# ziyanx02/multiagent-quadruped-environment

Measured on AMD Instinct MI355X. Metric: env-steps/sec (agents x envs x steps/s), go1gate 4096 envs x 2 agents per GPU, higher is better.
Workload: dtype f32 (policy GEMMs and the actuator network's 32 x 32 layer: 2-plane split-f16, 22-bit); 1 GPU; go1gate, 2 agents, num_envs=4096 per GPU (4096 total), 4 substeps x 5 ms per step; parallelism=single GPU

## Files before the change

### multiagent-quadruped-environment_amd/csrc/kernels_physics.hpp

```cpp
#pragma once
#include "mqe_common.hpp"

struct V3 { float x, y, z; };
__device__ __forceinline__ V3 v3(float x, float y, float z) { V3 r; r.x = x; r.y = y; r.z = z; return r; }
__device__ __forceinline__ V3 operator+(V3 a, V3 b) { return v3(a.x + b.x, a.y + b.y, a.z + b.z); }
__device__ __forceinline__ V3 operator-(V3 a, V3 b) { return v3(a.x - b.x, a.y - b.y, a.z - b.z); }
__device__ __forceinline__ V3 operator*(float s, V3 a) { return v3(s * a.x, s * a.y, s * a.z); }
__device__ __forceinline__ float dot(V3 a, V3 b) { return a.x * b.x + a.y * b.y + a.z * b.z; }
__device__ __forceinline__ V3 cross(V3 a, V3 b) { return v3(a.y * b.z - a.z * b.y, a.z * b.x - a.x * b.z, a.x * b.y - a.y * b.x); }
__device__ __forceinline__ V3 ld3(const float* p) { return v3(p[0], p[1], p[2]); }
__device__ __forceinline__ void st3(float* p, V3 a) { p[0] = a.x; p[1] = a.y; p[2] = a.z; }
__device__ __forceinline__ V3 mat_vec(const float* R, V3 v) {
  return v3(R[0] * v.x + R[1] * v.y + R[2] * v.z, R[3] * v.x + R[4] * v.y + R[5] * v.z, R[6] * v.x + R[7] * v.y + R[8] * v.z);
}
__device__ __forceinline__ V3 sym_vec(const float* S, V3 v) {
  return v3(S[0] * v.x + S[3] * v.y + S[4] * v.z, S[3] * v.x + S[1] * v.y + S[5] * v.z, S[4] * v.x + S[5] * v.y + S[2] * v.z);
}

template <int CTRL> __device__ __forceinline__ float dpp_take(float x) {
  return __int_as_float(__builtin_amdgcn_update_dpp(0, __float_as_int(x), CTRL, 0xF, 0xF, true));
}
__device__ __forceinline__ float lane_next(float x) { return dpp_take<0x130>(x); }
__device__ __forceinline__ float lane_prev(float x) { return dpp_take<0x138>(x); }

// ... 208 lines not shown
  float4* c4 = reinterpret_cast<float4*>(cr);
  c4[0] = make_float4(__int_as_float(a), __int_as_float(linkA), __int_as_float(b), __int_as_float(linkB));
  c4[1] = make_float4(p.x, p.y, p.z, sd);
  c4[2] = make_float4(n.x, n.y, n.z, __int_as_float(repA));
  c4[3] = make_float4(0.0f, 0.0f, 0.0f, __int_as_float(repB));
}

__host__ __device__ inline int mqe_maxc_uncapped(int A, int P, int cap_npc) { return 8 * A + cap_npc * P + (A + P > 4 ? 8 : 0); }
__host__ __device__ inline int mqe_maxc(int A, int P, int cap_npc) { const int v = mqe_maxc_uncapped(A, P, cap_npc); return v > 64 ? 64 : v; }
#define MQE_LIMIT_PASSES 4
#define CAP_ROBOT 8

struct PhysLds {
  int root, dof, tau, body, rhs, acc, acth, fcol, leg, legc, basei, sinv, sph, prim, con, side, phi, srec, wacc, total;
};
#define RS_STRIDE 44
#define RS_SLOT 12
#define RS_BIAS 42
#define RS_USN 43
#define RSB_STRIDE 32
#define RSB_INFO 30
__host__ __device__ inline int mqe_maxpair(int maxc) { return maxc / 2; }
__host__ __device__ inline PhysLds phys_lds_layout(int A, int P, int ND, int nbody, int ndof, int nsph, int nprim, int maxc, int rowgs, int pad) {
  const int BODY_STRIDE = BODY_STRIDE_OF(pad), CON_STRIDE = CON_STRIDE_OF(pad);
  PhysLds L; int o = 0;
  L.root = o; o += (A + P) * 13;
  L.dof = o; o += ND * 2;
  L.tau = o; o += 12 * A;
  o = (o + 3) & ~3;
  L.rhs = o; o += (ndof + 3) & ~3;
  L.acc = o; o += (ndof + 3) & ~3;
  L.acth = o; o += 4 * 12 * A;
  L.leg = o; o += A * 4 * LEG_STRIDE;
  L.sinv = o; o += A * 72;
  L.con = o; o += maxc * CON_STRIDE;
  L.body = o; o += nbody * BODY_STRIDE;
  L.phi = L.body; L.srec = L.phi;
  if (rowgs && L.phi + maxc * RS_STRIDE > o) o = L.phi + maxc * RS_STRIDE;
  const int scratch = o;
  L.fcol = o; o += A * 5 * FCOL_STRIDE;
  L.legc = o; o += A * 4 * LEGC_STRIDE;
  L.basei = o; o += A * 24;
  L.sph = scratch; L.prim = scratch + nsph * 4;
  if (L.prim + nprim * 8 > o) o = L.prim + nprim * 8;
  L.side = scratch;
  if (scratch + mqe_maxpair(maxc) * RSB_STRIDE > o) o = scratch + mqe_maxpair(maxc) * RSB_STRIDE;
  L.wacc = scratch + mqe_maxpair(maxc) * RSB_STRIDE;
  if (L.wacc + ((ndof + 3) & ~3) > o) o = L.wacc + ((ndof + 3) & ~3);
  L.total = o;
  return L;
}

__host__ __device__ inline int post_npc_stride(int P) { return (P * 13 + 3) & ~3; }
__host__ __device__ inline int post_staging_floats(int epw, int amp, int nj, int P) { return epw * amp * (MQE_OBS_BAG + 24) + epw * post_npc_stride(P) + epw * nj; }
struct PhysDebug { float* minv; int* nc; float* contacts; int robot; long long* times; int stop_after; };
#define TSTAMP(i) do { if (dbg.times != nullptr && lane == 0) dbg.times[i] = (long long)wall_clock64(); if (dbg.stop_after == (i)) return; } while (0)

enum { PS_LOAD_STATE = 1, PS_LOAD_TAU = 2, PS_STORE_STATE = 4, PS_WRITE_CF = 8 };

enum { PS_F_LINK = 1, PS_F_NPC = 2, PS_F_BOX = 4, PS_F_STATIC = 8,
       PS_F_FEW = 16,
       PS_F_ROW = 32 };
template <int TP> struct ShapeClass {
  static constexpr bool small = TP == 0 || TP == PS_F_LINK || (TP > 0 && (TP & PS_F_FEW) != 0);
  static constexpr int sweep = TP >= 0 ? 1 : -1;
  static constexpr int npq = (small || (TP > 0 && (TP & PS_F_ROW) != 0)) ? 2 : 4;
};
template <int TA, int TP>
struct PhysShape {
  const int A, P, PD, npcdof, ND, nbody, ndof, maxc, n_static;
  const bool has_seesaw, has_box;
  const bool rowgs;
  __device__ __forceinline__ explicit PhysShape(const DevModel* m)
      : A(TA > 0 ? TA : m->A), P(TP == 0 ? 0 : m->P), PD((TP < 0 || (TP & PS_F_NPC)) ? m->n_npc_dyn : 0),
        npcdof((TP < 0 || (TP & PS_F_NPC)) ? m->npc_dofs_each : 0),
        ND((TA > 0 && TP == 0) ? 12 * TA : m->ND), nbody((TA > 0 && TP == 0) ? TA * MQE_NBODY : m->nbody_env),
        ndof((TA > 0 && TP == 0) ? TA * MQE_RD : m->ndof_env), maxc((TA > 0 && TP == 0) ? mqe_maxc(TA, 0, 2) : m->maxc),
        n_static((TP < 0 || (TP & PS_F_STATIC)) ? m->n_static : 0),
        has_seesaw(TP < 0 ? m->has_seesaw != 0 : (TP & PS_F_LINK) != 0), has_box(TP < 0 ? m->has_box != 0 : (TP & PS_F_BOX) != 0),
        rowgs(ShapeClass<TP>::sweep >= 0 ? ShapeClass<TP>::sweep == 1 : m->rowgs != 0) {}
};

template <int TA, int TP, int EPW = 1, bool LATE = false>
__device__ __forceinline__ void phys_substep(const DevModel* __restrict__ m, const DevState& st, float* lds_wave, const int e_first, const int lane_wave,
                                             const int flags, const int no_write, const PhysDebug& dbg, const int hotv,
                                             const DevModel* mtab = nullptr) {
  static_assert(EPW == 1 || (EPW == 2 && TP == 0 && (TA == 1 || TA == 2)), "two envs per wavefront: robot-only scenes of at most two robots");
  auto HI = [&](int i) -> int { return __builtin_amdgcn_readlane(hotv, i); };
  auto HF = [&](int i) -> float { return __int_as_float(__builtin_amdgcn_readlane(hotv, i)); };
  auto HP = [&](int i) -> const float* {
    return as_global(reinterpret_cast<const float*>(((unsigned long long)(unsigned)__builtin_amdgcn_readlane(hotv, i + 1) << 32) | (unsigned long long)(unsigned)__builtin_amdgcn_readlane(hotv, i)));
  };
  auto HMASK = [&]() -> unsigned long long {
    return ((unsigned long long)(unsigned)__builtin_amdgcn_readlane(hotv, HOT_FEAT_MASK_HI) << 32) | (unsigned long long)(unsigned)__builtin_amdgcn_readlane(hotv, HOT_FEAT_MASK_LO);
  };
  constexpr int LW = 64 / EPW;
  const int grp = EPW == 1 ? 0 : lane_wave / LW;
  const int lane = EPW == 1 ? lane_wave : lane_wave - grp * LW;
  const bool evalid = EPW == 1 || e_first + grp < HI(HOT_N);
  const int e = evalid ? e_first + grp : HI(HOT_N) - 1;
  auto gballot = [&](bool p) -> unsigned long long {
    const unsigned long long b = __ballot(p);
    return EPW == 1 ? b : ((b >> (grp * LW)) & ((1ull << (LW & 63)) - 1ull));
  };
  auto wave_max_of_groups = [&](int x) -> int {
    return EPW == 1 ? x : max(__builtin_amdgcn_readlane(x, 0), __builtin_amdgcn_readlane(x, 32));
  };
// ... 1947 lines not shown
        if (ok && h == 0) {
          acthg[nj + jt] = he1; acthg[jt] = err; acthg[3 * nj + jt] = hv1; acthg[2 * nj + jt] = qd;
          ldsg[L.tau + jt] = tau;
          if (ev) {
            ST_LATE(late, st, sub_tau)[((size_t)eg * 4 + (k < 4 ? k : 3)) * nj + jt] = tau;
            if (last) ST_LATE(late, st, torques)[gi] = tau;
            if (lagged) ST_LATE(late, st, lag_buf)[lag_wr] = as;
          }
        }
      }
    }
    __syncthreads();
    if constexpr (TIMED) {
      long long* tt = ST_LATE(late, st, wave_times) + 4 * (size_t)gridDim.x + ((size_t)blockIdx.x * 4 + (k < 4 ? k : 3)) * 16;
      const PhysDebug tdbg = {nullptr, nullptr, nullptr, 0, tt, -1};
      phys_substep<TA, TP, EPW, late>(mk, st, lds_wave, e_first_k, lane_k, last ? (PS_STORE_STATE | PS_WRITE_CF) : 0, 0, tdbg, hotv, ma);
      if (lane_wave == 0) tt[15] = (long long)wall_clock64();
    } else
    phys_substep<TA, TP, EPW, late>(mk, st, lds_wave, e_first_k, lane_k, last ? (PS_STORE_STATE | PS_WRITE_CF) : 0, 0, nodbg, hotv, ma);
    if (evalid)
      for (int jt = glane_k; jt < nj; jt += LW) {
        const float q = lds[L.dof + jt * 2], qd = lds[L.dof + jt * 2 + 1];
        substep_log(ma, ST_LATE(late, st, sub_dof_vel), ST_LATE(late, st, sub_exceed), ((size_t)e_k * 4 + (k < 4 ? k : 3)) * nj + jt, jt % 12, q, qd);
      }
  }
  __syncthreads();
  const int lane_post = late ? lane_wave : lane_run;
  const int lane_pg = EPW == 1 ? lane_post : lane_post - (lane_post / LW) * LW;
  if constexpr (late) {
    st = late_state();
    asm volatile("" : "+s"(e_first_k));
  }
  const int e_post = EPW == 1 ? e_first_k : e;
  if (evalid)
    for (int i = lane_pg; i < 4 * nj; i += LW) {
      const int w = i / nj, jt = i - w * nj;
      st.act_hist[(size_t)w * R12 + (size_t)e_post * nj + jt] = acth[i];
    }
  if constexpr (ShapeClass<TP>::small || TP > 0) if (pa.on) {
    long long* et = nullptr;
    if constexpr (TIMED) { et = st.wave_times + 68 * (size_t)gridDim.x + (size_t)blockIdx.x * 16; if (lane_post == 0) et[0] = (long long)wall_clock64(); }
    __threadfence_block();
    __syncthreads();
    constexpr int AMP = (TA == 1 || TA == 2) ? 2 : MQE_MAX_AGENTS;
    float* sb = lds_wave + L.body;
    float* act_l = sb + EPW * AMP * (MQE_OBS_BAG + 24) + EPW * post_npc_stride(P);
    for (int i = lane_post; i < EPW * nj; i += 64) {
      const int ge = i / nj, jt = i - ge * nj;
      if (e_first + ge < m->N) act_l[ge * nj + jt] = st.actions[(size_t)(e_first + ge) * nj + jt];
    }
    __syncthreads();
    if constexpr (TIMED) { if (lane_post == 0) et[1] = (long long)wall_clock64(); }
    post_body<AMP, EPW, true>(m, st, (int)blockIdx.x, lane_post, sb, sb + EPW * AMP * MQE_OBS_BAG, sb + EPW * AMP * (MQE_OBS_BAG + 24), pa.wrapper_level, pa.push_count, pa.step_no,
                        lds_wave + L.root, lds_wave + L.dof, act_l, L.total, nj, post_npc_stride(P), et);
    if constexpr (TIMED) { if (lane_post == 0) et[10] = (long long)wall_clock64(); }
  }
  if (st.wave_times && lane_post == 0) st.wave_times[4 * blockIdx.x + 1] = (long long)wall_clock64();
}
```

### multiagent-quadruped-environment_amd/csrc/kernels_step.hpp

```cpp
#pragma once
#include <type_traits>
#include "mqe_common.hpp"

__device__ __forceinline__ void quat_rotate_inverse_f(const float* q, const float* v, float* o) {
  float qw = q[3];
  float s = 2.0f * qw * qw - 1.0f;
  float cx = q[1] * v[2] - q[2] * v[1], cy = q[2] * v[0] - q[0] * v[2], cz = q[0] * v[1] - q[1] * v[0];
  float dt = q[0] * v[0] + q[1] * v[1] + q[2] * v[2];
  o[0] = v[0] * s - cx * qw * 2.0f + q[0] * dt * 2.0f;
  o[1] = v[1] * s - cy * qw * 2.0f + q[1] * dt * 2.0f;
  o[2] = v[2] * s - cz * qw * 2.0f + q[2] * dt * 2.0f;
}
__device__ __forceinline__ float wrap2pi(float a) {
  const float T = 6.2831855f;
  float r = fmodf(a, T);
  if (r < 0) r += T;
  return r;
}
__device__ __forceinline__ void euler_xyz_f(const float* q, float* rpy) {
  float x = q[0], y = q[1], z = q[2], w = q[3];
  float sinr = 2.0f * (w * x + y * z), cosr = w * w - x * x - y * y + z * z;
  float sinp = 2.0f * (w * y - z * x);
  float siny = 2.0f * (w * z + x * y), cosy = w * w + x * x - y * y - z * z;
  float roll = atan2f(sinr, cosr);
// ... 482 lines not shown
typedef const __attribute__((address_space(3))) float* lds_cptr;
template <class NP>
__device__ __forceinline__ void sheep_flock_mean(const DevModel* m, NP npc_rows, float* avg) {
  const int P = m->P;
  avg[0] = 0; avg[1] = 0; avg[2] = 0;
  for (int p = 0; p < P; p++) for (int k = 0; k < 3; k++) avg[k] += npc_rows[p * 13 + k];
  for (int k = 0; k < 3; k++) avg[k] /= (float)P;
}
template <class NP>
__device__ __forceinline__ void sheep_flock_stats(const DevModel* m, const DevState& st, int e, NP npc_rows, const float* avg) {
  const int P = m->P;
  float var = 0;
  for (int k = 0; k < 2; k++) {
    float acc = 0;
    for (int p = 0; p < P; p++) { float t = npc_rows[p * 13 + k] - avg[k]; acc += t * t; }
    var += acc / (float)P;
  }
  st.sheep_avg[e * 2] = avg[0]; st.sheep_avg[e * 2 + 1] = avg[1];
  st.sheep_var[e] = var;
}
template <class NP, class RP>
__device__ __forceinline__ void sheep_increment(const DevModel* m, const DevState& st, int e, int p, NP npc_rows, RP rob_rows, const float* avg, int step_no, float* dv) {
  const int A = m->A, P = m->P;
  NP sp = npc_rows + p * 13;
  for (int k = 0; k < 3; k++) {
    const float z = m->noise_mode == MQE_NOISE_SCRIPTED ? st.npc_noise[((size_t)e * P + p) * 3 + k]
                                                        : (m->sheep_rand != 0.0f ? mqe_randn(m, e, step_no, (uint32_t)(p * 3 + k)) : 0.0f);
    dv[k] = m->sheep_rand * z * 2.0f;
  }
  if (P != 1) {
    float rel[3] = {avg[0] - sp[0], avg[1] - sp[1], avg[2] - sp[2]};
    float nr = sqrtf(rel[0] * rel[0] + rel[1] * rel[1] + rel[2] * rel[2]);
    if (nr > 0.0f) for (int k = 0; k < 3; k++) dv[k] += m->sheep_rand * rel[k] / nr / 1.5f;
  }
  for (int a = 0; a < A; a++) {
    RP dp = rob_rows + a * 13;
    float rel[3] = {sp[0] - dp[0], sp[1] - dp[1], sp[2] - dp[2]};
    float sq[3] = {rel[0] * rel[0], rel[1] * rel[1], rel[2] * rel[2]};
    float dis = sqrtf(sq[0] * sq[0] + sq[1] * sq[1] + sq[2] * sq[2]);
    float den = powf(dis, 1.4f);
    for (int k = 0; k < 3; k++) { float t = rel[k] / den; if (dis > 9.0f) t = 0.0f; dv[k] += m->sheep_scale * t; }
  }
  dv[2] = 0.0f;
}
template <class NP>
__device__ __forceinline__ void sheep_apply(float* root, int A, int p, NP npc_rows, const float* dv) {
  float* sp = root + (A + p) * 13;
  NP old = npc_rows + p * 13;
  const float v0 = clampf(old[7] + dv[0], -2.0f, 2.0f), v1 = clampf(old[8] + dv[1], -2.0f, 2.0f), v2 = old[9] + dv[2];
  sp[7] = v0; sp[8] = v1; sp[9] = v2;
  sp[2] = clampf(old[2], 0.0f, 0.3f);
  sp[3] = 0.0f; sp[4] = 0.0f;
}
template <bool BAG_LDS = false>
__device__ __forceinline__ void wrapper_env_dev(const DevModel* m, const DevState& st, int e, int is_reset_call, const float* npc, int side_effects = 1, const float* bag_in = nullptr) {
  typedef typename std::conditional<BAG_LDS, const __attribute__((address_space(3))) float*, const float*>::type bag_ptr;
  bag_ptr bag;
  if constexpr (BAG_LDS) bag = (bag_ptr)bag_in;
  else bag = bag_in ? bag_in : st.obs_bag + (size_t)e * m->A * MQE_OBS_BAG;
  int A = m->A, P = m->P, Aw = m->Aw, D = m->D;
  const int task = m->task;
  float* obs = st.wobs + (size_t)e * Aw * D;
  float* rew = st.wrew + (size_t)e * Aw;
  float* rs = st.rsum + (size_t)e * MQE_MAX_REWARD_TERMS;
  float sc[7];
#pragma unroll
  for (int k = 0; k < 7; k++) sc[k] = m->reward_scale[k];
  const bool early = task == MQE_TASK_GATE || task == MQE_TASK_SHEEP || task == MQE_TASK_SEESAW || task == MQE_TASK_PUSHBOX || task == MQE_TASK_FOOTBALL_DEFENDER;
  float gp0 = 0.0f, gp1 = 0.0f, eol[3] = {0.0f, 0.0f, 0.0f}, eo0 = 0.0f, eo1 = 0.0f;
  if (task == MQE_TASK_GATE || task == MQE_TASK_SHEEP || task == MQE_TASK_PUSHBOX || (task == MQE_TASK_FOOTBALL_DEFENDER && !is_reset_call && (sc[0] != 0 || sc[1] != 0))) {
    gp0 = as_global(m->gate_pos)[e * 2]; gp1 = as_global(m->gate_pos)[e * 2 + 1];
  }
  if (task == MQE_TASK_PUSHBOX || task == MQE_TASK_FOOTBALL_DEFENDER)
    for (int k = 0; k < 3; k++) eol[k] = st.env_origins_live[e * 3 + k];
  if (task == MQE_TASK_SHEEP) { eo0 = as_global(m->env_origins)[e * 3]; eo1 = as_global(m->env_origins)[e * 3 + 1]; }
  if (early) {
    if (is_reset_call) { for (int a = 0; a < Aw; a++) rew[a] = 0; }
    else {
      float r_env = 0.0f;
      uint8_t was_reset = st.reset_buf[e];
      float rsv[7];
#pragma unroll
      for (int k = 0; k < 7; k++) rsv[k] = rs[k];
      if (task == MQE_TASK_GATE) {
        float r_ag[MQE_MAX_AGENTS] = {0, 0, 0, 0}, bx[MQE_MAX_AGENTS] = {0, 0, 0, 0}, by[MQE_MAX_AGENTS] = {0, 0, 0, 0}, wl[MQE_MAX_AGENTS] = {0, 0, 0, 0};
        const uint8_t have = st.w_have_last[e];
        const float gx = gp0, colf = (float)st.collide_buf[e];
        float rs0 = rsv[0], rs1 = rsv[1], rs2 = rsv[2], rs3 = rsv[3];
        const float wp0 = m->wrapper_param[0], wp1 = m->wrapper_param[1];
#pragma unroll
        for (int a = 0; a < MQE_MAX_AGENTS; a++)
          if (a < A) {
            bag_ptr ob = bag + (a) * MQE_OBS_BAG;
            bx[a] = ob[0]; by[a] = ob[1];
            wl[a] = st.w_last[e * MQE_MAX_AGENTS + a];
          }
        float tsum = 0;
#pragma unroll
        for (int a = 0; a < MQE_MAX_AGENTS; a++)
          if (a < A) {
            const float tx = wp0, ty = (a == 0 ? 1.0f : -1.0f) * wp1;
            const float dist = sqrtf((bx[a] - tx) * (bx[a] - tx) + (by[a] - ty) * (by[a] - ty));
            const float last = have ? wl[a] : dist;
            tsum += last - dist;
            st.w_last[e * MQE_MAX_AGENTS + a] = dist;
          }
        st.w_have_last[e] = 1;
// ... 66 lines not shown
        for (int a = 0; a < MQE_MAX_AGENTS; a++) if (a < A) wl[a] = st.w_last[e * MQE_MAX_AGENTS + a];
#pragma unroll
        for (int a = 0; a < MQE_MAX_AGENTS; a++)
          if (a < A) {
            bag_ptr ob = bag + (a) * MQE_OBS_BAG;
            const float x = ob[0];
            xs += x - (have ? wl[a] : x);
            st.w_last[e * MQE_MAX_AGENTS + a] = x;
            zs += ob[2]; y2 += ob[1] * ob[1];
          }
        st.w_have_last[e] = 1;
        if (sc[0] != 0) { if (was_reset) xs = 0; xs *= sc[0]; r_env += xs; rsv[0] += xs; }
        if (sc[1] != 0) { float v = sc[1] * (zs - 0.56f); r_env += v; rsv[1] += v; }
        if (sc[2] != 0) { float v = sc[2] * (y2 - 0.5f); r_env += v; rsv[2] += v; }
        if (sc[3] != 0) { float v = sc[3] * colf; r_env += v; rsv[3] += v; }
        if (sc[4] != 0) {
          bag_ptr o0 = bag; bag_ptr o1 = bag + (A - 1) * MQE_OBS_BAG;
          float d2 = (o0[0] - o1[0]) * (o0[0] - o1[0]) + (o0[1] - o1[1]) * (o0[1] - o1[1]);
          if (d2 < 0.25f) { float v = div_ieee(sc[4], d2); r_env += v; rsv[4] += v; }
        }
        if (sc[5] != 0) {
          int cnt = 0;
          for (int a = 0; a < A; a++) { bag_ptr ob = bag + (a) * MQE_OBS_BAG; if (ob[0] > 7.7f && ob[2] > 1.3f) cnt++; }
          float v = sc[5] * (float)cnt; r_env += v; rsv[5] += v;
        }
        if (fell) { r_env += sc[6]; rsv[6] += sc[6]; }
        for (int a = 0; a < Aw; a++) rew[a] = r_env;
      } else if (task == MQE_TASK_PUSHBOX) {
        const float bx = npc[0] - eol[0], wl20 = st.w_last2[e * 2];
        const uint8_t have = st.w_have_last[e];
        if (sc[0] != 0 && have) {
          float xm = bx - wl20;
          if (was_reset) xm = 0;
          const float v = sc[0] * xm;
          r_env += v; rsv[0] += v;
        }
        st.w_last2[e * 2] = bx;
        st.w_have_last[e] = 1;
        for (int a = 0; a < Aw; a++) rew[a] = r_env;
      } else if (task == MQE_TASK_FOOTBALL_DEFENDER) {
        float bx = npc[0] - eol[0], by = npc[1] - eol[1];
        if (sc[0] != 0) { if (bx > gp0) { r_env += sc[0]; rsv[0] += sc[0]; } }
        if (sc[1] != 0) {
          float dg = sqrtf((bx - gp0) * (bx - gp0) + (by - gp1) * (by - gp1));
          float v = sc[1] * expf(-dg / 3.0f);
          r_env += v; rsv[1] += v;
        }
        for (int a = 0; a < Aw; a++) rew[a] = r_env;
      }
#pragma unroll
      for (int k = 0; k < 7; k++) rs[k] = rsv[k];
    }
  }
  for (int a = 0; a < Aw; a++) {
    float* o = obs + a * D;
    int c = 0;
    if (task == MQE_TASK_TUG) {
      const float npos = st.dof[((size_t)e * m->ND + 12 * A) * 2], nvel = st.dof[((size_t)e * m->ND + 12 * A) * 2 + 1];
      const float sgn = a == 1 ? -1.0f : 1.0f;
      bag_ptr ob = bag + (a) * MQE_OBS_BAG;
      float v6[6];
      for (int k = 0; k < 6; k++) v6[k] = ob[k];
      const float dx = v6[0] - 1.6f, dy = v6[1] - npos;
      v6[1] *= sgn; v6[4] *= sgn;
      for (int k = 0; k < 6; k++) o[k] = v6[k];
      o[6] = sgn * npos; o[7] = nvel; o[8] = sqrtf(dx * dx + dy * dy); o[9] = sgn * npos;
      continue;
    }
    if (task != MQE_TASK_ROTATION && task != MQE_TASK_BRIDGE && task != MQE_TASK_WRESTLING)
      for (int k = 0; k < Aw; k++) o[c++] = (k == a) ? 1.0f : 0.0f;
    bag_ptr ob = bag + (a) * MQE_OBS_BAG;
    for (int k = 0; k < 6; k++) o[c++] = ob[k];
    if (task != MQE_TASK_PLAIN) {
      bag_ptr ob2 = bag + ((Aw - 1 - a)) * MQE_OBS_BAG;
      for (int k = 0; k < 6; k++) o[c++] = ob2[k];
    }
    if (task == MQE_TASK_GATE || task == MQE_TASK_SHEEP || task == MQE_TASK_PUSHBOX) { o[c++] = gp0; o[c++] = gp1; }
    if (task == MQE_TASK_PUSHBOX) {
      o[c++] = npc[0] - eol[0]; o[c++] = npc[1] - eol[1];
      for (int k = 0; k < 4; k++) o[c++] = npc[3 + k];
    }
    if (task == MQE_TASK_SHEEP)
      for (int p = 0; p < P; p++) { o[c++] = npc[p * 13] - eo0; o[c++] = npc[p * 13 + 1] - eo1; }
    if (task == MQE_TASK_FOOTBALL_DEFENDER) {
      for (int k = 0; k < 3; k++) o[c++] = npc[k] - eol[k];
      for (int k = 0; k < 3; k++) o[c++] = npc[7 + k];
    }
  }
  if (early) return;
  if (task == MQE_TASK_TUG) {
    float* nd = st.dof + ((size_t)e * m->ND + 12 * A) * 2;
    const float npos = nd[0];
    bag_ptr ob0 = bag;
    bag_ptr ob1 = bag + (1) * MQE_OBS_BAG;
    const float x0 = ob0[0], y0 = ob0[1], x1 = ob1[0], y1 = ob1[1];
    if (is_reset_call) {
      st.w_last[e * MQE_MAX_AGENTS] = x0; st.w_last[e * MQE_MAX_AGENTS + 1] = y0;
      st.w_last2[e * 2] = npos;
      st.w_delayed_reset[e] = 0;
      for (int a = 0; a < Aw; a++) rew[a] = 0;
      return;
    }
    const float last_npc = st.w_last2[e * 2];
    const float lx = st.w_last[e * MQE_MAX_AGENTS] - 1.6f, ly = st.w_last[e * MQE_MAX_AGENTS + 1] - npos;
    const float cx = x0 - 1.6f, cy = y0 - npos;
    const float last_dis = sqrtf(lx * lx + ly * ly), dis = sqrtf(cx * cx + cy * cy);
    float r0 = 0.0f, sr = 0.0f, pu = 0.0f, pr = 0.0f, pp = 0.0f;
    if (sc[0] != 0) { if (npos < 0) sr = sc[0] * -npos; if (last_npc <= npos) sr /= 2; r0 += sr; rs[0] += sr; }
    if (sc[1] != 0) { if (npos > 0) pu = sc[1] * npos; if (last_npc > npos) pu /= 2; r0 -= pu; rs[1] += pu; }
    if (sc[2] != 0) { if (dis < last_dis) pr = (last_dis - dis) * sc[2]; r0 += pr; rs[2] += pr; }
    if (sc[3] != 0) { if (dis >= last_dis) pp = powf(2.0f, dis) * sc[3]; r0 -= pp; rs[3] += pp; }
    rs[4] += npos; rs[5] += pr + sr - pu; rs[6] += x0; rs[7] += y0; rs[8] += x1; rs[9] += y1;
    st.w_last[e * MQE_MAX_AGENTS] = x0; st.w_last[e * MQE_MAX_AGENTS + 1] = y0;
    st.w_last2[e * 2] = npos;
    rew[0] = r0;
    for (int a = 1; a < Aw; a++) rew[a] = 0;
    if (side_effects) {
      uint8_t cnt = st.reset_buf[e] ? 2 : st.w_delayed_reset[e];
      if (cnt > 0) { nd[0] = 0.0f; nd[1] = 0.0f; cnt--; }
      st.w_delayed_reset[e] = cnt;
    }
    return;
  }
  if (task == MQE_TASK_BRIDGE) {
    bag_ptr ob0 = bag;
    bag_ptr ob1 = bag + (1) * MQE_OBS_BAG;
    const float x0 = ob0[0], z0 = ob0[2], x1 = ob1[0], z1 = ob1[2];
    float S = st.w_last[e * MQE_MAX_AGENTS], tgt = st.w_last[e * MQE_MAX_AGENTS + 1];
    if (is_reset_call) {
      S = fabsf(x1 + x0); tgt = x1;
      st.w_last[e * MQE_MAX_AGENTS] = S; st.w_last[e * MQE_MAX_AGENTS + 1] = tgt;
    }
    float* o1 = obs + 1 * D;
    o1[0] = S - o1[0]; o1[4] = -o1[4]; o1[6] = S - o1[6]; o1[10] = -o1[10];
    if (is_reset_call) { for (int a = 0; a < Aw; a++) rew[a] = 0; return; }
    float r0 = 0.0f;
    if (sc[0] != 0 && z1 < 0.5f) { r0 += sc[0]; rs[0] += sc[0]; }
    if (sc[1] != 0 && z0 < 0.5f) { r0 -= sc[1]; rs[1] += sc[1]; }
    if (sc[2] != 0 && x0 > tgt) { r0 += sc[2]; rs[2] += sc[2]; }
    rew[0] = r0;
    for (int a = 1; a < Aw; a++) rew[a] = 0;
    return;
  }
  if (task == MQE_TASK_WRESTLING) {
    float* o1 = obs + 1 * D;
    o1[1] = -o1[1]; o1[4] = -o1[4]; o1[7] = -o1[7]; o1[10] = -o1[10];
    if (is_reset_call) { for (int a = 0; a < Aw; a++) rew[a] = 0; return; }
    float r0 = 0.0f;
    bool down0, down1;
    {
      bag_ptr ob = bag;
      float r = ob[3], p = ob[4];
      if (r > 3.1415927f) r -= 6.2831855f;
      if (p > 3.1415927f) p -= 6.2831855f;
      down0 = fabsf(p) > 3.1415927f * 0.9f || fabsf(r) >= 3.1415927f * 0.4f;
      ob += MQE_OBS_BAG;
      r = ob[3]; p = ob[4];
      if (r > 3.1415927f) r -= 6.2831855f;
      if (p > 3.1415927f) p -= 6.2831855f;
      down1 = fabsf(p) > 3.1415927f * 0.9f || fabsf(r) >= 3.1415927f * 0.4f;
    }
    if (sc[0] != 0 && down1) { r0 += sc[0]; rs[0] += sc[0]; }
    if (sc[1] != 0 && down0) { r0 -= sc[1]; rs[1] += sc[1]; }
    rew[0] = r0;
    for (int a = 1; a < Aw; a++) rew[a] = 0;
    return;
  }
  if (task == MQE_TASK_ROTATION) {
    float* o1 = obs + 1 * D;
    o1[1] = -o1[1]; o1[4] = -o1[4]; o1[7] = -o1[7]; o1[10] = -o1[10];
    const float tgt = m->wrapper_param[0];
    bag_ptr ob0 = bag;
    bag_ptr ob1 = bag + (1) * MQE_OBS_BAG;
    const float x0 = ob0[0], y0 = ob0[1], x1 = ob1[0];
    if (is_reset_call) {
      st.w_last[e * MQE_MAX_AGENTS] = sqrtf((x0 - tgt) * (x0 - tgt) + y0 * y0);
      for (int a = 0; a < Aw; a++) rew[a] = 0;
      return;
    }
    float r0 = 0.0f;
    if (sc[0] != 0 && x0 > tgt) { r0 += sc[0]; rs[0] += sc[0]; }
    if (sc[1] != 0 && x1 > tgt) { r0 -= sc[1]; rs[1] += sc[1]; }
    if (sc[2] != 0) {
      const float dis = sqrtf((x0 - tgt) * (x0 - tgt) + (y0 - tgt) * (y0 - tgt));
      if (dis < st.w_last[e * MQE_MAX_AGENTS]) { r0 += sc[2]; rs[2] += sc[2]; }
      st.w_last[e * MQE_MAX_AGENTS] = dis;
    }
    rew[0] = r0;
    for (int a = 1; a < Aw; a++) rew[a] = 0;
    return;
  }
  for (int a = 0; a < Aw; a++) rew[a] = 0;
}

#ifndef POST_EPW
#define POST_EPW 8
#endif

__device__ __forceinline__ void post_flush_rows(float* __restrict__ g, const float* lds, const int n, const int tid) {
  const int n4 = n >> 2;
  for (int i = tid; i < n4; i += 64) reinterpret_cast<float4*>(g)[i] = reinterpret_cast<const float4*>(lds)[i];
  for (int i = (n4 << 2) + tid; i < n; i += 64) g[i] = lds[i];
}

template <int AM, int PEPW, bool LDS_STATE = false>
__device__ __forceinline__ void post_body(const DevModel* m, const DevState& st, const int blk, const int tid, float* s_bag, float* s_la, float* s_npc,
                                          int wrapper_level, int push_count, int step_no,
                                          const float* root_l = nullptr, const float* dof_l = nullptr, const float* act_l = nullptr, int lds_env_stride = 0, int act_env_stride = 0,
                                          const int npc_stride = MQE_MAX_NPCS * 13, long long* taps = nullptr) {
  static_assert(PEPW * AM <= 64 && (PEPW & (PEPW - 1)) == 0, "agent lanes of PEPW envs must fit one wavefront");
#define ETAP(i) do { if (taps != nullptr && tid == 0) taps[i] = (long long)wall_clock64(); } while (0)
  const int A = m->A, P = m->P;
  const int le = tid & (PEPW - 1), a = tid / PEPW;
  const int e = blk * PEPW + le;
  const bool mine = e < m->N && a < A;
  const bool lead = e < m->N && a == 0;
  const int i = e * A + a;
  const int nrow = min(PEPW, m->N - blk * PEPW) * A;
  const float dtp = m->dt * (float)m->decimation;
  float* root = st.root + (size_t)e * (A + P) * 13;
  float* bag = s_bag + le * A * MQE_OBS_BAG;
  typedef typename std::conditional<LDS_STATE, lds_cptr, const float*>::type state_ptr;
  state_ptr root_src;
  if constexpr (LDS_STATE) root_src = (lds_cptr)(root_l + le * lds_env_stride); else root_src = root;
  float* la = s_la + le * A * 12;
  float rs[13], gpar[5], gi0 = 0.f, f3[3], aoz = 0.f, dq[24], act[12], eo[3];
  int ep = 0;
  if (mine) {
    ep = st.ep_len[e] + 1;
#pragma unroll
    for (int k = 0; k < 3; k++) eo[k] = as_global(m->env_origins)[e * 3 + k];
#pragma unroll
    for (int k = 0; k < 13; k++) rs[k] = root_src[a * 13 + k];
    const float* lo = st.loco_obs + (size_t)i * MQE_FRAME;
#pragma unroll
    for (int k = 0; k < 5; k++) gpar[k] = lo[7 + k];
    gi0 = st.gait[i];
    const float* cf3 = st.cf + ((size_t)e * m->NBR + a * MQE_NREP) * 3;
#pragma unroll
    for (int k = 0; k < 3; k++) f3[k] = cf3[k];
    aoz = as_global(m->agent_origins)[(size_t)i * 3 + 2];
    state_ptr ds, as;
    if constexpr (LDS_STATE) { ds = (lds_cptr)(dof_l + le * lds_env_stride + a * 24); as = (lds_cptr)(act_l + le * act_env_stride + a * 12); }
    else { ds = st.dof + ((size_t)e * m->ND + a * 12) * 2; as = st.actions + (size_t)i * 12; }
#pragma unroll
    for (int k = 0; k < 24; k++) dq[k] = ds[k];
#pragma unroll
    for (int k = 0; k < 12; k++) act[k] = as[k];
  }
  float bq[4], lv[3], av[3], pgr[3], clk[4], gi1 = 0.f;
  float rpy[3] = {0.f, 0.f, 0.f};
  unsigned fl = 0;
  if (mine) {
#pragma unroll
    for (int k = 0; k < 4; k++) bq[k] = rs[3 + k];
    fl = robot_frame(m, rs, gpar, gi0, f3, aoz, dtp, lv, av, pgr, clk, gi1, rpy);
  }
  ETAP(2);
#pragma unroll
  for (int d = PEPW; d < PEPW * AM; d <<= 1) fl |= (unsigned)__shfl_xor((int)fl, d);
  const uint8_t to = ep > m->max_episode_length;
  const uint8_t reset = (uint8_t)(mine && (fl != 0 || to));
  if (lead) env_flags_store(m, st, e, ep, fl, to, reset);
  if (mine) robot_frame_store(st, i, lv, av, pgr, bq, clk, gi1);
  ETAP(3);
  float* npc_pre = s_npc + le * npc_stride;
  {
    const int e0 = blk * PEPW, nenv = min(PEPW, m->N - e0), per = P * 13;
    for (int t = tid; t < nenv * per; t += 64) {
      const int sl = t / per, r = t - sl * per;
      if constexpr (LDS_STATE) s_npc[sl * npc_stride + r] = ((lds_cptr)(root_l + sl * lds_env_stride))[A * 13 + r];
      else s_npc[sl * npc_stride + r] = st.root[((size_t)(e0 + sl) * (A + P) + A) * 13 + r];
    }
    __syncthreads();
  }
  ETAP(4);
  if (m->npc_kind == MQE_NPC_SHEEP) {
    constexpr int LPE = 64 / PEPW, NPASS = (MQE_MAX_NPCS + LPE - 1) / LPE;
    float dvs[NPASS][3];
    if (e < m->N) {
      float avg[3];
      sheep_flock_mean(m, (lds_cptr)npc_pre, avg);
      if (lead) sheep_flock_stats(m, st, e, (lds_cptr)npc_pre, avg);
#pragma unroll
      for (int q = 0; q < NPASS; q++)
        if (a + q * LPE < P) sheep_increment(m, st, e, a + q * LPE, (lds_cptr)npc_pre, root_src, avg, step_no, dvs[q]);
    }
    __syncthreads();
    if (e < m->N) {
#pragma unroll
      for (int q = 0; q < NPASS; q++)
        if (a + q * LPE < P) sheep_apply(root, A, a + q * LPE, (lds_cptr)npc_pre, dvs[q]);
    }
    __threadfence_block();
    __syncthreads();
  }
  ETAP(5);
  if (lead) {
    if (reset) {
      reset_env_dev(m, st, e);
      for (int k = 0; k < P * 13; k++) npc_pre[k] = root[A * 13 + k];
    }
  }
  if (__ballot(reset != 0)) {
    __threadfence_block();
    __syncthreads();
    if (reset) {
#pragma unroll
      for (int k = 0; k < 13; k++) rs[k] = root[a * 13 + k];
      const float* ds = st.dof + ((size_t)e * m->ND + a * 12) * 2;
#pragma unroll
      for (int k = 0; k < 24; k++) dq[k] = ds[k];
      if (P == 0) {
#pragma unroll
        for (int k = 0; k < 4; k++) { bq[k] = rs[3 + k]; st.bquat[i * 4 + k] = bq[k]; }
        euler_xyz_f(bq, rpy);
      }
    }
  }
  ETAP(6);
  if (mine) {
    float* ob = bag + a * MQE_OBS_BAG;
#pragma unroll
    for (int k = 0; k < 3; k++) obs_row_axis(ob, k, rs[k], eo[k], rpy[k], lv[k], av[k], pgr[k]);
#pragma unroll
    for (int j = 0; j < 12; j++) obs_row_joint(m, ob, j, dq[2 * j], dq[2 * j + 1], act[j], act[j]);
#pragma unroll
    for (int k = 0; k < 4; k++) obs_row_quad(ob, k, clk[k], bq[k]);
#pragma unroll
    for (int k = 71; k < MQE_OBS_BAG; k++) ob[k] = 0.0f;
#pragma unroll
    for (int j = 0; j < 12; j++) {
      la[a * 12 + j] = act[j];
      la[PEPW * AM * 12 + a * 12 + j] = dq[2 * j + 1];
    }
  }
  __syncthreads();
  ETAP(7);
  if (lead) {
    wrapper_env_dev<true>(m, st, e, 0, npc_pre, wrapper_level, bag);
    if (push_count > 0 && !reset) push_robots(m, root, e, A, push_count);
  }
  ETAP(8);
  {
    const size_t r0 = (size_t)blk * PEPW * A;
    post_flush_rows(st.obs_bag + r0 * MQE_OBS_BAG, s_bag, nrow * MQE_OBS_BAG, tid);
    post_flush_rows(st.last_actions + r0 * 12, s_la, nrow * 12, tid);
    post_flush_rows(st.last_dof_vel + r0 * 12, s_la + PEPW * AM * 12, nrow * 12, tid);
  }
  ETAP(9);
  unsigned long long rm = __ballot(lead && reset != 0);
  while (rm) {
    const int l = __ffsll((long long)rm) - 1;
    rm &= rm - 1;
    zero_env_history(m, st, blk * PEPW + l, tid, 64);
  }
}

template <int AM>
__global__ void __launch_bounds__(64) k_post_physics(const DevModel* m, DevState st, int wrapper_level, int push_count, int step_no) {
  __shared__ float4 s_bag4[POST_EPW * AM * MQE_OBS_BAG / 4], s_la4[POST_EPW * AM * 24 / 4];
  __shared__ float s_npc[POST_EPW * MQE_MAX_NPCS * 13];
  post_body<AM, POST_EPW>(m, st, blockIdx.x, threadIdx.x, reinterpret_cast<float*>(s_bag4), reinterpret_cast<float*>(s_la4), s_npc, wrapper_level, push_count, step_no);
}

__global__ void k_reset_history(const DevModel* m, DevState st) {
  int idx = blockIdx.x * blockDim.x + threadIdx.x;
  int i = idx / HIST_F4;
  if (i >= m->R) return;
  if (!st.reset_buf[i / m->A]) return;
  reinterpret_cast<float4*>(st.hist)[idx] = make_float4(0.f, 0.f, 0.f, 0.f);
  if (st.hist2) {
    const int w = idx - i * HIST_F4;
    if (w < HIST2_U4) reinterpret_cast<uint4*>(st.hist2)[(size_t)i * HIST2_U4 + w] = make_uint4(0u, 0u, 0u, 0u);
    if (w == 0) st.hist_irr[i] = 0u;
  }
}

__global__ void k_hist2_rebuild(const DevModel* m, DevState st, int oldest) {
  const int idx = blockIdx.x * blockDim.x + threadIdx.x;
  const int i = idx / MQE_HIST, slot = idx - i * MQE_HIST;
  if (i >= m->R || !st.hist2) return;
  const float* fr = st.hist + ((size_t)i * MQE_HIST + slot) * MQE_FRAME;
  uint16_t* row2 = st.hist2 + (size_t)i * (2 * MQE_HIST * MQE_H2_FRAME);
  unsigned any = 0u;
  for (int c = 0; c < 70; c++) {
    const float v = fr[c];
    any |= __float_as_uint(v) & 0x7FFFFFFFu;
    const int cc = h2_col(c);
    if (cc >= 0) {
      uint16_t h, l;
      split2(v, MQE_H2_ASCALE, h, l);
      const size_t k = (size_t)slot * MQE_H2_FRAME + cc;
// ... 96 lines not shown
```

### multiagent-quadruped-environment_amd/csrc/mqe_common.hpp

```cpp
#pragma once
#include <hip/hip_runtime.h>
#include <stdint.h>
#include <string.h>
#include <stddef.h>
#include <type_traits>

#include "../../include/mqe_hip.h"

#define MQE_RD 18
#define MQE_OBS_BAG 74
#define MQE_WAVE 64

struct DevMlp {
  int n_layers;
  int dims[MQE_MAX_LAYERS + 1];
  const float* W[MQE_MAX_LAYERS];
  const float* b[MQE_MAX_LAYERS];
};

struct DevModel {
  int N, A, P, R, ND, NBR, Aw, D;
  int npc_kind, task, npc_dofs_each, npc_lin_only, n_npc_dyn;
  int env_id_offset, seed, noise_mode;
  float dt; int decimation; float gravity_z; int solver_iterations;
  float contact_offset, max_depen, friction, erp;
  int solver_type, vel_iters;
  mqe_robot_model robot;
  float npc_mass, npc_inertia; int npc_n_spheres; float npc_sphere_center[8][3]; float npc_sphere_radius[8];
  int self_collision;
  int rowgs;
  int lag_steps; float max_push;
  int has_box, cap_npc; float npc_box_half[3];
  float seesaw_default_angle;
  int n_static; float sb_center[4][3], sb_half[4][3];
  int has_seesaw, ss_axis, ss_link_cyl; float ss_joint_offset[3], ss_plank_center[3], ss_plank_half[3], ss_base_half[3];
  float ss_inertia, ss_vel_limit, ss_col_radius, ss_col_length, ss_theta_lo, ss_theta_hi;
  int control_type; float action_scale, hip_scale_reduction, clip_actions; float torque_limits[12]; float kp, kd;
  float default_dof_pos[12]; float command_obs[70]; float cmd_lin_scale, cmd_ang_scale; int clip_command;
  int cmd_dims, cmd_general; int cmd_src[18]; float cmd_scale[18];
  const float* wall_sdf; int sdf_nx, sdf_ny; float hs, wall_height, ground_z;
  const float* wall_top;
  const float* wall_corner;
  int edge_mask;
  float prim_feat_t[MQE_MAX_PRIMS][2];
  const float* ground_height;
  float soft_lo[12], soft_hi[12];
  const float *env_origins, *agent_origins, *base_init, *npc_init, *gate_pos;
  int curriculum, terrain_rows, terrain_cols; float terrain_env_length;
  const float* terrain_origins; const int32_t* terrain_types;
  int termination_flags, terminate_on_base_contact, max_episode_length;
  float roll_thr, pitch_thr, zlow_thr, zhigh_thr;
  float dof_ratio_lo, dof_ratio_hi; int has_base_pos_range, has_npc_pos_range;
  float base_pos_x_lo, base_pos_x_hi, base_pos_y_lo, base_pos_y_hi, npc_pos_x_lo, npc_pos_x_hi, npc_pos_y_lo, npc_pos_y_hi;
  float base_vel_lo, base_vel_hi;
  float sheep_scale, sheep_rand;
  float reward_scale[MQE_MAX_REWARD_TERMS]; float wrapper_param[8];
  uint32_t hot[64];
  DevMlp actuator;
  const float* act_frag;
  const uint16_t* act_frag16; int act_f16;
  int nbody_env, ndof_env, nsph_env, nprim_env, maxc;
  unsigned long long feat_sphere_mask;
};

// ... 225 lines not shown
```

Measured before the change: 40.19 million env-steps/s.

## Spread post-step observation rows and wrapper obs across all wavefront lanes

In the LDS-state post path, each agent lane now stashes its per-agent frame quantities into a small LDS record. Afterwards all 64 lanes build the observation-bag rows cooperatively, one axis, joint or quad row call per lane, instead of one agent lane doing every row. The wrapper's per-agent observation assembly is also moved out of the single lead lane into a lane-parallel function, and the lead lane skips that loop. This trades extra LDS staging, an added barrier and index arithmetic for removing the serial per-lane work that left most of the wavefront idle.

```diff
diff --git a/multiagent-quadruped-environment_amd/csrc/kernels_physics.hpp b/multiagent-quadruped-environment_amd/csrc/kernels_physics.hpp
--- a/multiagent-quadruped-environment_amd/csrc/kernels_physics.hpp
+++ b/multiagent-quadruped-environment_amd/csrc/kernels_physics.hpp
@@ -284,7 +284,8 @@
 }
 
 __host__ __device__ inline int post_npc_stride(int P) { return (P * 13 + 3) & ~3; }
-__host__ __device__ inline int post_staging_floats(int epw, int amp, int nj, int P) { return epw * amp * (MQE_OBS_BAG + 24) + epw * post_npc_stride(P) + epw * nj; }
+__host__ __device__ inline int post_rec_offset(int epw, int amp, int nj, int P) { return epw * amp * (MQE_OBS_BAG + 24) + epw * post_npc_stride(P) + epw * nj; }
+__host__ __device__ inline int post_staging_floats(int epw, int amp, int nj, int P) { return post_rec_offset(epw, amp, nj, P) + epw * amp * MQE_POST_REC; }
 struct PhysDebug { float* minv; int* nc; float* contacts; int robot; long long* times; int stop_after; };
 #define TSTAMP(i) do { if (dbg.times != nullptr && lane == 0) dbg.times[i] = (long long)wall_clock64(); if (dbg.stop_after == (i)) return; } while (0)
 
@@ -2338,7 +2339,7 @@
     __syncthreads();
     if constexpr (TIMED) { if (lane_post == 0) et[1] = (long long)wall_clock64(); }
     post_body<AMP, EPW, true>(m, st, (int)blockIdx.x, lane_post, sb, sb + EPW * AMP * MQE_OBS_BAG, sb + EPW * AMP * (MQE_OBS_BAG + 24), pa.wrapper_level, pa.push_count, pa.step_no,
-                        lds_wave + L.root, lds_wave + L.dof, act_l, L.total, nj, post_npc_stride(P), et);
+                        lds_wave + L.root, lds_wave + L.dof, act_l, L.total, nj, post_npc_stride(P), et, sb + post_rec_offset(EPW, AMP, nj, P));
     if constexpr (TIMED) { if (lane_post == 0) et[10] = (long long)wall_clock64(); }
   }
   if (st.wave_times && lane_post == 0) st.wave_times[4 * blockIdx.x + 1] = (long long)wall_clock64();
diff --git a/multiagent-quadruped-environment_amd/csrc/kernels_step.hpp b/multiagent-quadruped-environment_amd/csrc/kernels_step.hpp
--- a/multiagent-quadruped-environment_amd/csrc/kernels_step.hpp
+++ b/multiagent-quadruped-environment_amd/csrc/kernels_step.hpp
@@ -558,7 +558,7 @@
   sp[2] = clampf(old[2], 0.0f, 0.3f);
   sp[3] = 0.0f; sp[4] = 0.0f;
 }
-template <bool BAG_LDS = false>
+template <bool BAG_LDS = false, bool OBS_ON_LANES = false>
 __device__ __forceinline__ void wrapper_env_dev(const DevModel* m, const DevState& st, int e, int is_reset_call, const float* npc, int side_effects = 1, const float* bag_in = nullptr) {
   typedef typename std::conditional<BAG_LDS, const __attribute__((address_space(3))) float*, const float*>::type bag_ptr;
   bag_ptr bag;
@@ -731,7 +731,7 @@
       for (int k = 0; k < 7; k++) rs[k] = rsv[k];
     }
   }
-  for (int a = 0; a < Aw; a++) {
+  for (int a = 0; a < (OBS_ON_LANES ? 0 : Aw); a++) {
     float* o = obs + a * D;
     int c = 0;
     if (task == MQE_TASK_TUG) {
@@ -811,7 +811,7 @@
       st.w_last[e * MQE_MAX_AGENTS] = S; st.w_last[e * MQE_MAX_AGENTS + 1] = tgt;
     }
     float* o1 = obs + 1 * D;
-    o1[0] = S - o1[0]; o1[4] = -o1[4]; o1[6] = S - o1[6]; o1[10] = -o1[10];
+    if constexpr (!OBS_ON_LANES) { o1[0] = S - o1[0]; o1[4] = -o1[4]; o1[6] = S - o1[6]; o1[10] = -o1[10]; }
     if (is_reset_call) { for (int a = 0; a < Aw; a++) rew[a] = 0; return; }
     float r0 = 0.0f;
     if (sc[0] != 0 && z1 < 0.5f) { r0 += sc[0]; rs[0] += sc[0]; }
@@ -823,7 +823,7 @@
   }
   if (task == MQE_TASK_WRESTLING) {
     float* o1 = obs + 1 * D;
-    o1[1] = -o1[1]; o1[4] = -o1[4]; o1[7] = -o1[7]; o1[10] = -o1[10];
+    if constexpr (!OBS_ON_LANES) { o1[1] = -o1[1]; o1[4] = -o1[4]; o1[7] = -o1[7]; o1[10] = -o1[10]; }
     if (is_reset_call) { for (int a = 0; a < Aw; a++) rew[a] = 0; return; }
     float r0 = 0.0f;
     bool down0, down1;
@@ -847,7 +847,7 @@
   }
   if (task == MQE_TASK_ROTATION) {
     float* o1 = obs + 1 * D;
-    o1[1] = -o1[1]; o1[4] = -o1[4]; o1[7] = -o1[7]; o1[10] = -o1[10];
+    if constexpr (!OBS_ON_LANES) { o1[1] = -o1[1]; o1[4] = -o1[4]; o1[7] = -o1[7]; o1[10] = -o1[10]; }
     const float tgt = m->wrapper_param[0];
     bag_ptr ob0 = bag;
     bag_ptr ob1 = bag + (1) * MQE_OBS_BAG;
@@ -872,9 +872,67 @@
   for (int a = 0; a < Aw; a++) rew[a] = 0;
 }
 
+template <int PEPW>
+__device__ __forceinline__ void wrapper_obs_lanes(const DevModel* m, const DevState& st, const int blk, const int tid, const float* s_bag, const float* s_npc, const int npc_stride) {
+  static_assert(PEPW <= 2 && MQE_MAX_AGENTS == 4, "env and agent of an element are found by comparisons");
+  const int A = m->A, P = m->P, Aw = m->Aw, D = m->D, task = m->task;
+  const int e0 = blk * PEPW, nenv = min(PEPW, m->N - e0), per = Aw * D;
+  const bool mirrored = task == MQE_TASK_ROTATION || task == MQE_TASK_BRIDGE || task == MQE_TASK_WRESTLING;
+  const int c_own = mirrored ? 0 : Aw, c_other = c_own + 6, c_task = task == MQE_TASK_PLAIN ? c_other : c_other + 6;
+  for (int idx = tid; idx < nenv * per; idx += 64) {
+    const int sl = (PEPW > 1 && idx >= per) ? 1 : 0;
+    const int i2 = idx - sl * per;
+    const int a = (i2 >= D ? 1 : 0) + (i2 >= 2 * D ? 1 : 0) + (i2 >= 3 * D ? 1 : 0);
+    const int c = i2 - a * D, e = e0 + sl;
+    lds_cptr bag = (lds_cptr)(s_bag + sl * A * MQE_OBS_BAG);
+    lds_cptr npc = (lds_cptr)(s_npc + sl * npc_stride);
+    float v = 0.0f;
+    bool have = true;
+    if (task == MQE_TASK_TUG) {
+      const float* nd = st.dof + ((size_t)e * m->ND + 12 * A) * 2;
+      const float npos = nd[0], sgn = a == 1 ? -1.0f : 1.0f;
+      lds_cptr ob = bag + a * MQE_OBS_BAG;
+      if (c < 6) { v = ob[c]; if (c == 1 || c == 4) v *= sgn; }
+      else if (c == 6 || c == 9) v = sgn * npos;
+      else if (c == 7) v = nd[1];
+      else if (c == 8) { const float dx = ob[0] - 1.6f, dy = ob[1] - npos; v = sqrtf(dx * dx + dy * dy); }
+      else have = false;
+    } else if (c < c_own) v = (c == a) ? 1.0f : 0.0f;
+    else if (c < c_task) {
+      v = c < c_other ? bag[a * MQE_OBS_BAG + (c - c_own)] : bag[(Aw - 1 - a) * MQE_OBS_BAG + (c - c_other)];
+      if (mirrored && a == 1) {
+        if (task == MQE_TASK_BRIDGE) {
+          if (c == 0 || c == 6) v = st.w_last[e * MQE_MAX_AGENTS] - v;
+          else if (c == 4 || c == 10) v = -v;
+        } else if (c == 1 || c == 4 || c == 7 || c == 10) v = -v;
+      }
+    } else {
+      int k = c - c_task;
+      have = false;
+      if (task == MQE_TASK_GATE || task == MQE_TASK_SHEEP || task == MQE_TASK_PUSHBOX) {
+        if (k < 2) { v = as_global(m->gate_pos)[e * 2 + k]; have = true; }
+        k -= 2;
+      }
+      if (!have && task == MQE_TASK_PUSHBOX) {
+        if (k < 2) { v = npc[k] - st.env_origins_live[e * 3 + k]; have = true; }
+        else if (k < 6) { v = npc[3 + (k - 2)]; have = true; }
+      }
+      if (!have && task == MQE_TASK_SHEEP && k < 2 * P) { v = npc[(k >> 1) * 13 + (k & 1)] - as_global(m->env_origins)[e * 3 + (k & 1)]; have = true; }
+      if (!have && task == MQE_TASK_FOOTBALL_DEFENDER) {
+        if (k < 3) { v = npc[k] - st.env_origins_live[e * 3 + k]; have = true; }
+        else if (k < 6) { v = npc[7 + (k - 3)]; have = true; }
+      }
+    }
+    if (have) st.wobs[(size_t)e * per + i2] = v;
+  }
+}
+
 #ifndef POST_EPW
 #define POST_EPW 8
 #endif
+
+struct PostRec { enum { EO = 0, POS = 3, RPY = 6, LV = 9, AV = 12, PG = 15, CLK = 18, BQ = 22, USED = 26 }; };
+static_assert(PostRec::USED <= MQE_POST_REC && MQE_POST_REC % 4 == 0, "the record keeps the staging area's 16 B granules");
 
 __device__ __forceinline__ void post_flush_rows(float* __restrict__ g, const float* lds, const int n, const int tid) {
   const int n4 = n >> 2;
@@ -886,8 +944,10 @@
 __device__ __forceinline__ void post_body(const DevModel* m, const DevState& st, const int blk, const int tid, float* s_bag, float* s_la, float* s_npc,
                                           int wrapper_level, int push_count, int step_no,
                                           const float* root_l = nullptr, const float* dof_l = nullptr, const float* act_l = nullptr, int lds_env_stride = 0, int act_env_stride = 0,
-                                          const int npc_stride = MQE_MAX_NPCS * 13, long long* taps = nullptr) {
+                                          const int npc_stride = MQE_MAX_NPCS * 13, long long* taps = nullptr,
+                                          float* s_rec = nullptr) {
   static_assert(PEPW * AM <= 64 && (PEPW & (PEPW - 1)) == 0, "agent lanes of PEPW envs must fit one wavefront");
+  static_assert(!LDS_STATE || PEPW <= 2, "the element lanes find their env by one comparison");
 #define ETAP(i) do { if (taps != nullptr && tid == 0) taps[i] = (long long)wall_clock64(); } while (0)
   const int A = m->A, P = m->P;
   const int le = tid & (PEPW - 1), a = tid / PEPW;
@@ -919,13 +979,14 @@
 #pragma unroll
     for (int k = 0; k < 3; k++) f3[k] = cf3[k];
     aoz = as_global(m->agent_origins)[(size_t)i * 3 + 2];
-    state_ptr ds, as;
-    if constexpr (LDS_STATE) { ds = (lds_cptr)(dof_l + le * lds_env_stride + a * 24); as = (lds_cptr)(act_l + le * act_env_stride + a * 12); }
-    else { ds = st.dof + ((size_t)e * m->ND + a * 12) * 2; as = st.actions + (size_t)i * 12; }
-#pragma unroll
-    for (int k = 0; k < 24; k++) dq[k] = ds[k];
-#pragma unroll
-    for (int k = 0; k < 12; k++) act[k] = as[k];
+    if constexpr (!LDS_STATE) {
+      const float* ds = st.dof + ((size_t)e * m->ND + a * 12) * 2;
+      const float* as = st.actions + (size_t)i * 12;
+#pragma unroll
+      for (int k = 0; k < 24; k++) dq[k] = ds[k];
+#pragma unroll
+      for (int k = 0; k < 12; k++) act[k] = as[k];
+    }
   }
   float bq[4], lv[3], av[3], pgr[3], clk[4], gi1 = 0.f;
   float rpy[3] = {0.f, 0.f, 0.f};
@@ -942,6 +1003,16 @@
   const uint8_t reset = (uint8_t)(mine && (fl != 0 || to));
   if (lead) env_flags_store(m, st, e, ep, fl, to, reset);
   if (mine) robot_frame_store(st, i, lv, av, pgr, bq, clk, gi1);
+  float* rec = LDS_STATE ? s_rec + (le * A + a) * MQE_POST_REC : nullptr;
+  if constexpr (LDS_STATE) if (mine) {
+#pragma unroll
+    for (int k = 0; k < 3; k++) {
+      rec[PostRec::EO + k] = eo[k]; rec[PostRec::POS + k] = rs[k]; rec[PostRec::RPY + k] = rpy[k];
+      rec[PostRec::LV + k] = lv[k]; rec[PostRec::AV + k] = av[k]; rec[PostRec::PG + k] = pgr[k];
+    }
+#pragma unroll
+    for (int k = 0; k < 4; k++) { rec[PostRec::CLK + k] = clk[k]; rec[PostRec::BQ + k] = bq[k]; }
+  }
   ETAP(3);
   float* npc_pre = s_npc + le * npc_stride;
   {
@@ -984,6 +1055,27 @@
   if (__ballot(reset != 0)) {
     __threadfence_block();
     __syncthreads();
+    if constexpr (LDS_STATE) {
+      if (reset) {
+#pragma unroll
+        for (int k = 0; k < 3; k++) rec[PostRec::POS + k] = root[a * 13 + k];
+        if (P == 0) {
+#pragma unroll
+          for (int k = 0; k < 4; k++) { bq[k] = root[a * 13 + 3 + k]; st.bquat[i * 4 + k] = bq[k]; rec[PostRec::BQ + k] = bq[k]; }
+          euler_xyz_f(bq, rpy);
+#pragma unroll
+          for (int k = 0; k < 3; k++) rec[PostRec::RPY + k] = rpy[k];
+        }
+      }
+      unsigned long long rd = __ballot(lead && reset != 0);
+      while (rd) {
+        const int l = __ffsll((long long)rd) - 1;
+        rd &= rd - 1;
+        const float* gd = st.dof + (size_t)(blk * PEPW + l) * m->ND * 2;
+        __attribute__((address_space(3))) float* ld = (__attribute__((address_space(3))) float*)(dof_l + l * lds_env_stride);
+        for (int t = tid; t < A * 24; t += 64) ld[t] = gd[t];
+      }
+    } else
     if (reset) {
 #pragma unroll
       for (int k = 0; k < 13; k++) rs[k] = root[a * 13 + k];
@@ -998,6 +1090,29 @@
     }
   }
   ETAP(6);
+  if constexpr (LDS_STATE) {
+    constexpr int ROW_CALLS = 20;
+    __syncthreads();
+    for (int idx = tid; idx < nrow * ROW_CALLS; idx += 64) {
+      const int r = idx / ROW_CALLS, w = idx - r * ROW_CALLS;
+      const int sl = (PEPW > 1 && r >= A) ? 1 : 0, ra = r - sl * A;
+      float* ob = s_bag + r * MQE_OBS_BAG;
+      lds_cptr rc = (lds_cptr)(s_rec + r * MQE_POST_REC);
+      if (w < 3) obs_row_axis(ob, w, rc[PostRec::POS + w], rc[PostRec::EO + w], rc[PostRec::RPY + w], rc[PostRec::LV + w], rc[PostRec::AV + w], rc[PostRec::PG + w]);
+      else if (w < 15) {
+        const int j = w - 3;
+        lds_cptr ds = (lds_cptr)(dof_l + sl * lds_env_stride + ra * 24);
+        const float q = ds[2 * j], qd = ds[2 * j + 1], ac = ((lds_cptr)(act_l + sl * act_env_stride + ra * 12))[j];
+        obs_row_joint(m, ob, j, q, qd, ac, ac);
+        s_la[r * 12 + j] = ac;
+        s_la[PEPW * AM * 12 + r * 12 + j] = qd;
+      } else if (w < 19) obs_row_quad(ob, w - 15, rc[PostRec::CLK + (w - 15)], rc[PostRec::BQ + (w - 15)]);
+      else {
+#pragma unroll
+        for (int k = 71; k < MQE_OBS_BAG; k++) ob[k] = 0.0f;
+      }
+    }
+  } else
   if (mine) {
     float* ob = bag + a * MQE_OBS_BAG;
 #pragma unroll
@@ -1016,8 +1131,9 @@
   }
   __syncthreads();
   ETAP(7);
+  if constexpr (LDS_STATE) wrapper_obs_lanes<PEPW>(m, st, blk, tid, s_bag, s_npc, npc_stride);
   if (lead) {
-    wrapper_env_dev<true>(m, st, e, 0, npc_pre, wrapper_level, bag);
+    wrapper_env_dev<true, LDS_STATE>(m, st, e, 0, npc_pre, wrapper_level, bag);
     if (push_count > 0 && !reset) push_robots(m, root, e, A, push_count);
   }
   ETAP(8);
diff --git a/multiagent-quadruped-environment_amd/csrc/mqe_common.hpp b/multiagent-quadruped-environment_amd/csrc/mqe_common.hpp
--- a/multiagent-quadruped-environment_amd/csrc/mqe_common.hpp
+++ b/multiagent-quadruped-environment_amd/csrc/mqe_common.hpp
@@ -10,6 +10,7 @@
 #define MQE_RD 18
 #define MQE_OBS_BAG 74
 #define MQE_WAVE 64
+#define MQE_POST_REC 28
 
 struct DevMlp {
   int n_layers;
```

Result: no change. 40.37 million env-steps/s (median of 6 runs) (+0.5%).
